# Z-yq/TensorflowASR

Hardware: AMD Instinct MI355X
Metric: audio-frames/sec/GPU + RTF, ConformerCTC(S) 10s utts, 1/2/4/8 MI355X (higher is better)
Workload: dtype f32

## Files before the change

### include/mi355asr.h

```cpp
#ifndef MI355ASR_H
#define MI355ASR_H

#include <stddef.h>
#include <stdint.h>

#ifdef __cplusplus
extern "C" {
#endif

#define MI355ASR_OK 0
#define MI355ASR_EINVAL -1
#define MI355ASR_ESTATE -2
#define MI355ASR_EWEIGHT -3
#define MI355ASR_EWORKSPACE -4
#define MI355ASR_EHIP -5

typedef struct mi355asr_model mi355asr_model;

typedef struct {
  int32_t dmodel;
  int32_t num_blocks;
  int32_t head_size;
  int32_t num_heads;
  int32_t kernel_size;
  float   fc_factor;
  int32_t reduction_factor;
  int32_t n_mels;
  int32_t sample_rate;
  int32_t stride_ms;
  int32_t n_dft;
  int32_t chunk_size;
  int32_t has_encoder;
  int32_t num_classes;
  int32_t ctc_num_blocks;
  int32_t ctc_kernel_size;
  float   ctc_fc_factor;
  int32_t gemm_dtype;
  int32_t mel_layer_type;
  int32_t add_wav_info;
} mi355asr_config;

const char* mi355asr_last_error(void);
const char* mi355asr_version(void);
int mi355asr_test_split_f16(const float* x_dev, int64_t n, uint16_t* hi_dev, uint16_t* lo_dev, void* stream);

int mi355asr_create(const mi355asr_config* cfg, mi355asr_model** out);
int mi355asr_destroy(mi355asr_model* m);

int mi355asr_load_weight(mi355asr_model* m, const char* name, const float* data_host, int32_t rank,
                         const int64_t* dims);
#define MI355ASR_DT_F32 0
#define MI355ASR_DT_F16 1
#define MI355ASR_DT_BF16 2
#define MI355ASR_DT_F64 3
#define MI355ASR_DT_I16 4
int mi355asr_load_weight_typed(mi355asr_model* m, const char* name, const void* data_host, int32_t dtype, int32_t rank,
                               const int64_t* dims);
int mi355asr_num_weights(const mi355asr_model* m);
const char* mi355asr_weight_name(const mi355asr_model* m, int32_t i);
int mi355asr_weight_shape(const mi355asr_model* m, int32_t i, int32_t* rank, int64_t* dims, int32_t max_rank);
int mi355asr_finalize_weights(mi355asr_model* m, void* stream);
int mi355asr_set_expected_rows(mi355asr_model* m, int64_t rows);
int mi355asr_stft_mode(const mi355asr_model* m);

int mi355asr_out_frames(const mi355asr_model* m, int32_t L, int32_t* mel_frames, int32_t* enc_frames);
int mi355asr_workspace_bytes(const mi355asr_model* m, int32_t B, int32_t L, size_t* bytes);
int mi355asr_ctc_workspace_bytes(const mi355asr_model* m, int32_t B, int32_t T, size_t* bytes);

int mi355asr_encoder_forward(mi355asr_model* m, const float* wav_dev, int32_t B, int32_t L, float* enc_out_dev,
                             void* ws_dev, size_t ws_bytes, void* stream);

int mi355asr_ctc_forward(mi355asr_model* m, const float* enc_dev, int32_t B, int32_t T, float* logits_dev,
                         int32_t* frame_argmax_dev, void* ws_dev, size_t ws_bytes, void* stream);

int mi355asr_ctc_greedy(const int32_t* frame_argmax_dev, const int32_t* in_len_dev, int32_t B, int32_t T,
                        int32_t blank, int32_t* ids_dev, int32_t* out_len_dev, void* stream);

// ... 249 lines not shown
```

### tensorflowasr_amd/_lib.py

```python
import ctypes
import os

_HERE = os.path.dirname(os.path.abspath(__file__))
LIB_PATH = os.environ.get("MI355ASR_LIB") or os.path.join(_HERE, "libmi355asr.so")


class Config(ctypes.Structure):
    _fields_ = [
        ("dmodel", ctypes.c_int32), ("num_blocks", ctypes.c_int32), ("head_size", ctypes.c_int32),
        ("num_heads", ctypes.c_int32), ("kernel_size", ctypes.c_int32), ("fc_factor", ctypes.c_float),
        ("reduction_factor", ctypes.c_int32), ("n_mels", ctypes.c_int32), ("sample_rate", ctypes.c_int32),
        ("stride_ms", ctypes.c_int32), ("n_dft", ctypes.c_int32), ("chunk_size", ctypes.c_int32),
        ("has_encoder", ctypes.c_int32), ("num_classes", ctypes.c_int32), ("ctc_num_blocks", ctypes.c_int32),
        ("ctc_kernel_size", ctypes.c_int32), ("ctc_fc_factor", ctypes.c_float), ("gemm_dtype", ctypes.c_int32),
        ("mel_layer_type", ctypes.c_int32), ("add_wav_info", ctypes.c_int32),
    ]


class ChunkConfig(ctypes.Structure):
    _fields_ = [(n, ctypes.c_int32) for n in ("dmodel", "head_size", "num_heads", "kernel_size")] + \
        [("fc_factor", ctypes.c_float)] + \
        [(n, ctypes.c_int32) for n in (
            "n_mels", "sample_rate", "stride_ms", "n_dft", "reduction_factor",
            "enc_num_blocks", "enc_win_front", "enc_win_back",
# ... 7 lines not shown
        [("fc_factor", ctypes.c_float), ("inp_classes", ctypes.c_int32), ("tar_classes", ctypes.c_int32)]


class VadConfig(ctypes.Structure):
    _fields_ = [(n, ctypes.c_int32) for n in ("dmodel", "frame", "decimate")]


class ChunkOutputs(ctypes.Structure):
    _fields_ = [(n, ctypes.c_void_p) for n in ("front_out", "enc_out", "picker_logits", "picker_hidden", "picked",
                                               "helper_out", "text_logits", "text_argmax")]


class ChunkStreamsOutputs(ctypes.Structure):
    _fields_ = [(n, ctypes.c_void_p) for n in ("phone_argmax", "n_picked", "text_argmax", "n_valid", "n_unvalid",
                                               "phone_logits", "text_logits", "picker_hidden")]


class BeamStreamsOutputs(ctypes.Structure):
    _fields_ = [(n, ctypes.c_void_p) for n in ("ids", "lens", "scores", "n_hyp", "frames", "status")]


class Mi355AsrError(RuntimeError):
    pass


_P = ctypes.c_void_p
_I = ctypes.c_int32
_SZ = ctypes.c_size_t

SIGNATURES = {
    "mi355asr_last_error": (ctypes.c_char_p, []),
    "mi355asr_version": (ctypes.c_char_p, []),
    "mi355asr_test_split_f16": (ctypes.c_int, [_P, ctypes.c_int64, _P, _P, _P]),
    "mi355asr_create": (ctypes.c_int, [ctypes.POINTER(Config), ctypes.POINTER(_P)]),
    "mi355asr_destroy": (ctypes.c_int, [_P]),
    "mi355asr_load_weight": (ctypes.c_int, [_P, ctypes.c_char_p, _P, _I, ctypes.POINTER(ctypes.c_int64)]),
    "mi355asr_load_weight_typed": (ctypes.c_int, [_P, ctypes.c_char_p, _P, _I, _I, ctypes.POINTER(ctypes.c_int64)]),
    "mi355asr_ctc_prefix_beam_workspace_bytes": (ctypes.c_int, [_I, _I, _I, _I, _I, ctypes.POINTER(ctypes.c_size_t)]),
    "mi355asr_frame_argmax": (ctypes.c_int, [_P, _I, _I, _P, _P]),
    "mi355asr_feature_pick_count": (ctypes.c_int, [_P, _I, _I, _I, _P, _P, _P, _P]),
    "mi355asr_feature_pick_gather": (ctypes.c_int, [_P, _P, _P, _P, _I, _I, _I, _I, _I, _P, _P, _P]),
    "mi355asr_num_weights": (ctypes.c_int, [_P]),
    "mi355asr_stft_mode": (ctypes.c_int, [_P]),
    "mi355asr_weight_name": (ctypes.c_char_p, [_P, _I]),
    "mi355asr_weight_shape": (ctypes.c_int, [_P, _I, ctypes.POINTER(ctypes.c_int32), ctypes.POINTER(ctypes.c_int64), _I]),
    "mi355asr_finalize_weights": (ctypes.c_int, [_P, _P]),
    "mi355asr_set_expected_rows": (ctypes.c_int, [_P, ctypes.c_int64]),
    "mi355asr_out_frames": (ctypes.c_int, [_P, _I, ctypes.POINTER(_I), ctypes.POINTER(_I)]),
    "mi355asr_workspace_bytes": (ctypes.c_int, [_P, _I, _I, ctypes.POINTER(_SZ)]),
    "mi355asr_ctc_workspace_bytes": (ctypes.c_int, [_P, _I, _I, ctypes.POINTER(_SZ)]),
    "mi355asr_encoder_forward": (ctypes.c_int, [_P, _P, _I, _I, _P, _P, _SZ, _P]),
    "mi355asr_ctc_forward": (ctypes.c_int, [_P, _P, _I, _I, _P, _P, _P, _SZ, _P]),
    "mi355asr_ctc_greedy": (ctypes.c_int, [_P, _P, _I, _I, _I, _P, _P, _P]),
    "mi355asr_ctc_loss_workspace_bytes": (ctypes.c_int, [_I, _I, _I, _I, _I, ctypes.POINTER(_SZ)]),
    "mi355asr_ctc_loss": (ctypes.c_int, [_P, _I, _P, _P, _P, _I, _I, _I, _I, _I, _P, _P, _P, _SZ, _P]),
    "mi355asr_ctc_align_workspace_bytes": (ctypes.c_int, [_I, _I, _I, _I, ctypes.POINTER(_SZ)]),
    "mi355asr_ctc_align": (ctypes.c_int, [_P, _I, _P, _P, _P, _I, _I, _I, _I, _I, _P, _P, _P, _P, _SZ, _P]),
    "mi355asr_ctc_prefix_beam_host": (ctypes.c_int, [_P, _P, _I, _I, _I, _I, ctypes.c_double, _I, _I, _I, _P, _P, _P, _P]),
    "mi355asr_ctc_prefix_beam": (ctypes.c_int, [_P, _I, _P, _I, _I, _I, _I, ctypes.c_double, _I, _I, _I, _P, _P, _P, _P,
                                                _P, _SZ, _P]),
    "mi355asr_beam_last_path": (_I, []),
    "mi355asr_beam_device_limits": (ctypes.c_int, [_I, ctypes.POINTER(_I), ctypes.POINTER(_I), ctypes.POINTER(_I), ctypes.POINTER(_I)]),
    "mi355asr_beam_math_eval": (ctypes.c_int, [_I, _P, _P, _I, _P]),
    "mi355asr_beam_create": (ctypes.c_int, [_I, _I, ctypes.c_double, _I, ctypes.POINTER(_P)]),
    "mi355asr_beam_decode": (ctypes.c_int, [_P, _P, _I, _I, _P, _P, _P, _P]),
    "mi355asr_beam_reset": (ctypes.c_int, [_P]),
# ... 84 lines not shown
```

### tensorflowasr_amd/csrc/api.hip

```cpp
#include "common.h"
#include "model.h"

namespace mi355 {


thread_local char g_err[512] = "";

int fail(int code, const char* fmt, ...) {
  va_list ap;
  va_start(ap, fmt);
  vsnprintf(g_err, sizeof(g_err), fmt, ap);
  va_end(ap);
  return code;
}

void same_pad(int n, int k, int s, int* out, int* before) {
  const int o = ceil_div(n, s);
  const int tot = std::max((o - 1) * s + k - n, 0);
  *out = o;
  *before = tot / 2;
}

int launch_mel_auto(const mi355asr_model* m, MelArgs& me, hipStream_t s) {
  if (m->mel_band) {
// ... 32 lines not shown
  p.amax = take(M);
  const int FT = ceil_div(F, 16);
  p.logp = take((size_t)Bp * F * m->dm.LP);
  p.pmax = take((size_t)Bp * std::max(FT * m->dm.NCH_dft, F));
  p.umax = take(Bp);
  p.mel = take((size_t)Bp * F * m->cfg.n_mels);
  p.sub = take(M * m->dm.F2 * d);
  p.wv_floats = wavpick_floats(m, Bp, F * m->dm.hop);
  p.wv = p.wv_floats ? take(p.wv_floats) : 0;
  p.total = lay.o;
  return p;
}


int geometry(const mi355asr_model* m, int B, int L, Geometry* g) {
  const auto& c = m->cfg;
  if (B <= 0 || L <= 0) return fail(MI355ASR_EINVAL, "B and L must be positive (B=%d, L=%d)", B, L);
  g->nblk = 1;
  g->Lb = L;
  if (c.chunk_size > 0) {
    if (L % c.chunk_size != 0)
      return fail(MI355ASR_EINVAL, "streaming encoder: L=%d is not a multiple of chunk_size=%d "
                  "(the reference reshapes [B,L,1]->[-1,chunk,1], conformer_blocks.py:585)", L, c.chunk_size);
    g->nblk = L / c.chunk_size;
    g->Lb = c.chunk_size;
  }
  g->Bp = B * g->nblk;
  g->F = ceil_div(g->Lb, m->dm.hop);
  g->T1 = ceil_div(g->F, m->dm.st1);
  g->T = ceil_div(g->T1, 2);
  return 0;
}


int run_mel(const mi355asr_model* m, const float* wav, int Bp, int Lb, int F, float* logp, float* pmax,
            float* umax, float* mel, hipStream_t s, const int32_t* wav_len = nullptr) {
  const auto& c = m->cfg;
  if (wav_len && (c.mel_layer_type != 0 || !m->fft_ok))
    return fail(MI355ASR_EINVAL, "ragged batches: the Melspectrogram frontend on the FFT STFT only (%s)",
                c.mel_layer_type == 1 ? "LEAF frontend" : c.mel_layer_type == 2 ? "Spectrogram layer" : "dense DFT STFT, stft_mode 0");
  if (c.mel_layer_type == 1) {
    int nf, pl;
    same_pad(Lb, 401, m->dm.hop, &nf, &pl);
    const int tile = m->leaf_terms ? kLeafSplitTile : 128, nrel = m->leaf_terms ? kLeafSplitSlots : 4;
    const int NH = ceil_div(Lb, tile);
    if (m->leaf_terms) {
      LeafConvArgs la{wav, m->leaf_wsplit, m->leaf_gcoef, logp, m->leaf_p0, m->leaf_p1, Bp, Lb, F, NH, m->dm.hop, pl};
      PROF(MI355ASR_K_STFT);
      LAUNCH_TRY(launch_leaf_conv_pool_split(m->leaf_terms, la, s), "leaf gabor conv (split bf16) + pooling");
    } else {
      LeafConvArgs la{wav, m->leaf_wp, m->leaf_gcoef, logp, m->leaf_p0, m->leaf_p1, Bp, Lb, F, NH, m->dm.hop, pl};
      PROF(MI355ASR_K_STFT);
      LAUNCH_TRY(launch_leaf_conv_pool(la, s), "leaf gabor conv + pooling");
    }
    LeafPcenArgs lp{logp, m->leaf_alpha, m->leaf_delta, m->leaf_root, m->leaf_smooth, m->leaf_gamma, m->leaf_beta, mel,
                    Bp, F, NH, m->dm.hop, pl, tile, nrel};
    { PROF(MI355ASR_K_MEL); LAUNCH_TRY(launch_leaf_pcen_norm(lp, s), "leaf PCEN + instance norm"); }
    return 0;
  }
  const int FT = ceil_div(F, 16);
  int out, before;
  same_pad(Lb, c.n_dft, m->dm.hop, &out, &before);
  StftArgs st{};
  st.wav = wav; st.logp = logp; st.pmax = pmax; st.wp = m->dft_wp;
  st.B = Bp; st.L = Lb; st.F = F; st.hop = m->dm.hop; st.pad_left = before; st.n_dft = c.n_dft;
  st.NT = m->dm.NT_dft; st.LP = m->dm.LP; st.nbins = m->dm.nbins; st.FT = FT; st.NCH = m->dm.NCH_dft;
  st.db10 = 1;
  int npart = FT * m->dm.NCH_dft;
  if (m->fft_ok) {
    FftStftArgs fa{wav, logp, pmax, m->fft_w1p, m->fft_w2p, m->fft_twc, m->fft_tws, m->fft_win,
                   Bp, Lb, F, m->dm.hop, before, m->dm.LP, 1};
    fa.w1s = m->fft_w1s; fa.w2s = m->fft_w2s; fa.w1h = m->fft_w1h; fa.w2h = m->fft_w2h;
    fa.wav_len = wav_len;
    { PROF(MI355ASR_K_STFT); LAUNCH_TRY(launch_fft_stft(fa, s), "stft (fft)"); }
    npart = F;
  } else {
    PROF(MI355ASR_K_STFT);
    LAUNCH_TRY(launch_stft(st, s), "stft");
  }
  UttMaxArgs um{pmax, umax, npart};
  um.wav_len = wav_len; um.hop = m->dm.hop;
  { PROF(MI355ASR_K_UTT_MAX); LAUNCH_TRY(launch_utt_max(um, Bp, s), "utterance max"); }
  MelArgs me{};
  me.logp = logp; me.umax = umax; me.mel = mel; me.wp = m->mel_wp;
  me.B = Bp; me.F = F; me.LP = m->dm.LP; me.nbins = m->dm.nbins; me.KBm = m->dm.KBm; me.NTm = m->dm.NTm;
  me.NM = c.n_mels; me.FT = FT; me.floor_db = -80.0f;
  if (c.mel_layer_type == 2) { PROF(MI355ASR_K_MEL); LAUNCH_TRY(launch_db_norm(me, s), "dB (Spectrogram layer)"); }
  else { PROF(MI355ASR_K_MEL); LAUNCH_TRY(launch_mel_auto(m, me, s), "dB + mel"); }
  return 0;
}

int run_subsampling(const mi355asr_model* m, const float* mel, int Bp, int F, float* sub, float* out,
                    hipStream_t s, bool mel_bounded, bool* defer_dense, const int32_t* wav_len) {
  if (defer_dense) *defer_dense = false;
  const auto& c = m->cfg;
  const int d = c.dmodel;
  int T1, pt1, T2, pt2;
  same_pad(F, 3, m->dm.st1, &T1, &pt1);
  same_pad(T1, 3, 2, &T2, &pt2);
  SubConvArgs sa{};
  sa.mel = mel; sa.out = sub;
  subconv_weights(m, sa, true);
  static const bool force_half = mi355_env("MI355ASR_SUBCONV_TERMS", -1) == 22;
  if (m->c2_whalf && (mel_bounded || force_half)) { sa.w2h = m->c2_whalf; sa.h_scale = m->c2_hscale; sa.h_wscale = m->c2_wscale; }
  if (sa.w2h && mel_bounded) { sa.c1_mscale = m->c1_mscale; sa.c1_wscale = m->c1_wscale; }
  sa.B = Bp; sa.F = F; sa.NM = c.n_mels; sa.T1 = T1; sa.F1 = m->dm.F1; sa.T2 = T2; sa.F2 = m->dm.F2;
// ... 244 lines not shown


}

thread_local int mi355asr_last_scheme = SCHEME_F32;

__global__ void split_f16_probe_kernel(const float* __restrict__ x, int64_t n, uint16_t* __restrict__ hi, uint16_t* __restrict__ lo) {
  const int64_t i = 2 * ((int64_t)blockIdx.x * blockDim.x + threadIdx.x);
  if (i >= n) return;
  const bool two = i + 1 < n;
  const float a = x[i], b = two ? x[i + 1] : 0.f;
  const unsigned h = split_hi_f16(a, b), l = split_lo_f16(h, a, b);
  hi[i] = (uint16_t)(h & 0xffffu);
  lo[i] = (uint16_t)(l & 0xffffu);
  if (two) {
    hi[i + 1] = (uint16_t)(h >> 16);
    lo[i + 1] = (uint16_t)(l >> 16);
  }
}

extern "C" {

const char* mi355asr_last_error(void) { return g_err; }
const char* mi355asr_version(void) { return "mi355asr 0.1 (gfx950, fp32 operands as fp16 pairs / bf16 triples on the MFMA pipe)"; }

int mi355asr_test_split_f16(const float* x_dev, int64_t n, uint16_t* hi_dev, uint16_t* lo_dev, void* stream) {
  if (!x_dev || !hi_dev || !lo_dev) return fail(MI355ASR_EINVAL, "null pointer");
  if (n < 1 || n > (int64_t)1 << 31) return fail(MI355ASR_EINVAL, "test_split_f16: need 1 <= n <= 2^31 (got %lld)", (long long)n);
  const int64_t pairs = (n + 1) / 2;
  hipLaunchKernelGGL(split_f16_probe_kernel, dim3((unsigned)((pairs + 255) / 256)), dim3(256), 0, (hipStream_t)stream, x_dev, n, hi_dev, lo_dev);
  return hipGetLastError() == hipSuccess ? MI355ASR_OK : fail(MI355ASR_EHIP, "test_split_f16: launch failed");
}

int mi355asr_create(const mi355asr_config* cfg, mi355asr_model** out) {
  if (!cfg || !out) return fail(MI355ASR_EINVAL, "null argument");
  mi355asr_config c = *cfg;
  if (c.mel_layer_type == 2) c.n_mels = c.n_dft / 2 + 1;
  if (c.dmodel != 144 && (c.dmodel % 128 != 0 || c.dmodel < 128 || c.dmodel > 1024))
    return fail(MI355ASR_EINVAL, "dmodel=%d: supported are 144 (ConformerS), 256 (ConformerM / StreamingS) and other multiples of 128 up to 1024 (512 = ConformerL)", c.dmodel);
  if (c.num_heads * c.head_size != c.dmodel)
    return fail(MI355ASR_EINVAL, "num_heads*head_size (%d*%d) must equal dmodel (%d)", c.num_heads, c.head_size, c.dmodel);
  if (!attention_head_size_ok(c.head_size))
    return fail(MI355ASR_EINVAL, "head_size=%d: attention kernels are instantiated for 12, 16, 24, 32, 36, 48, 64, 72 and 128", c.head_size);
  if (c.kernel_size < 1 || c.kernel_size > 1024)
    return fail(MI355ASR_EINVAL, "kernel_size=%d: must be in 1 .. 1024", c.kernel_size);
  if (c.num_classes > 0 && (c.ctc_kernel_size < 1 || c.ctc_kernel_size > 1024))
    return fail(MI355ASR_EINVAL, "ctc_kernel_size=%d: must be in 1 .. 1024", c.ctc_kernel_size);
  if (c.reduction_factor != 2 && c.reduction_factor != 4 && c.reduction_factor != 6 && c.reduction_factor != 8)
    return fail(MI355ASR_EINVAL, "reduction_factor=%d: 2, 4, 6 or 8 (conv1 time stride 1 .. 4)", c.reduction_factor);
  if (c.mel_layer_type < 0 || c.mel_layer_type > 2)
    return fail(MI355ASR_EINVAL, "mel_layer_type=%d: 0 (Melspectrogram), 1 (leaf) or 2 (Spectrogram)", c.mel_layer_type);
  if (c.mel_layer_type == 1 && (c.n_mels != 80 || c.stride_ms * c.sample_rate / 1000 != 160 || c.sample_rate != 16000))
    return fail(MI355ASR_EINVAL, "leaf frontend: instantiated for 80 filters, 16 kHz, 10 ms stride (window 401, hop 160)");
  if (c.gemm_dtype != 0 && c.gemm_dtype != 1) return fail(MI355ASR_EINVAL, "gemm_dtype=%d: 0 (fp32 MFMA) or 1 (bf16 MFMA)", c.gemm_dtype);
  if (c.n_dft != 1024) return fail(MI355ASR_EINVAL, "n_dft=%d: the reference hard-codes 1024 (conformer_blocks.py:312)", c.n_dft);
  if (c.mel_layer_type != 2 && c.n_mels != 80 && c.n_mels != 128)
    return fail(MI355ASR_EINVAL, "n_mels=%d: mel kernel instantiated for 80 and 128", c.n_mels);
  if (c.num_blocks < 0 || c.ctc_num_blocks < 0 || c.chunk_size < 0 || c.num_classes < 0)
    return fail(MI355ASR_EINVAL, "negative count in config");
  auto* m = new mi355asr_model();
  m->cfg = c;
  {
    const int t = (int)mi355_env("MI355ASR_LEAF_TERMS", -1);
    if (t == 0 || t == 2 || t == 3) m->leaf_terms = t;
  }
  Dims& dm = m->dm;
// ... 344 lines not shown
```

### tensorflowasr_amd/csrc/fft_stft.hip

```cpp
#include <cstdlib>
#include <type_traits>

#include "common.h"
#include "env.h"
#include "launch.h"

namespace {

constexpr int LDW = 36;

__global__ __launch_bounds__(BLOCK_THREADS, 2) void fft_stft_kernel(FftStftArgs a) {
  __shared__ float lds[WAVES_PER_BLOCK][2][32 * LDW];
  const int lane = threadIdx.x & 63;
  const int g = lane >> 4, g4 = g * 4, c = lane & 15;
  const int wave = threadIdx.x >> 6;
  float* Lre = lds[wave][0];
  float* Lim = lds[wave][1];
  const int wid = blockIdx.x * WAVES_PER_BLOCK + wave;
  const int nwaves = gridDim.x * WAVES_PER_BLOCK;
  const int total = a.B * a.F;

  const f32x4* __restrict__ w1p = reinterpret_cast<const f32x4*>(a.w1p) + lane;
  const f32x4* __restrict__ w2p = reinterpret_cast<const f32x4*>(a.w2p) + lane;
  f32x4 w1[2][4], w2[4][2];
// ... 152 lines not shown
}
DEV f32x4 mma32(u32x4_t a, u32x4_t b, f32x4 c) {
  return __builtin_amdgcn_mfma_f32_16x16x32_bf16(__builtin_bit_cast(bf16x8_t, a), __builtin_bit_cast(bf16x8_t, b), c, 0, 0, 0);
}
typedef _Float16 f16x8_t __attribute__((ext_vector_type(8)));
constexpr float kStageScale = 16384.f;
DEV Split8 split8h(f32x4 lo, f32x4 hi) {
  unsigned d0[4], d1[4];
  split8_f16(lo, hi, d0, d1);
  Split8 f;
  f.t[0] = u32x4_t{d0[0], d0[1], d0[2], d0[3]};
  f.t[1] = u32x4_t{d1[0], d1[1], d1[2], d1[3]};
  f.t[2] = u32x4_t{0u, 0u, 0u, 0u};
  return f;
}
DEV f32x4 mma32h(u32x4_t a, u32x4_t b, f32x4 c) {
  return __builtin_amdgcn_mfma_f32_16x16x32_f16(__builtin_bit_cast(f16x8_t, a), __builtin_bit_cast(f16x8_t, b), c, 0, 0, 0);
}
DEV float pow2_scale(float m) {
  const int e = (int)((__builtin_bit_cast(unsigned, m) >> 23) & 255u);
  return __builtin_bit_cast(float, (unsigned)(127 + min(100, max(-14, 140 - e))) << 23);
}
DEV float recip_pow2(float s) { return __builtin_bit_cast(float, 0x7f000000u - __builtin_bit_cast(unsigned, s)); }
DEV float max8(f32x4 a, f32x4 b) {
  return fmaxf(fmaxf(fmaxf(fabsf(a.x), fabsf(a.y)), fmaxf(fabsf(a.z), fabsf(a.w))), fmaxf(fmaxf(fabsf(b.x), fabsf(b.y)), fmaxf(fabsf(b.z), fabsf(b.w))));
}
template <int N> DEV float dpp_ror(float v) {
  return __builtin_bit_cast(float, __builtin_amdgcn_update_dpp(0, __builtin_bit_cast(int, v), 0x120 + N, 0xf, 0xf, false));
}
DEV float row_sum16(float v) { v += dpp_ror<8>(v); v += dpp_ror<4>(v); v += dpp_ror<2>(v); v += dpp_ror<1>(v); return v; }
DEV float row_max16(float v) {
  v = fmaxf(v, dpp_ror<8>(v)); v = fmaxf(v, dpp_ror<4>(v)); v = fmaxf(v, dpp_ror<2>(v)); return fmaxf(v, dpp_ror<1>(v));
}
DEV float col_max(float m) {
  return group_max(m);
}

#ifndef MI355ASR_STFT_DIAG
#define MI355ASR_STFT_DIAG 0
#endif
constexpr int FDG = MI355ASR_STFT_DIAG;
#ifndef MI355ASR_STFT_TABS_LDS
#define MI355ASR_STFT_TABS_LDS 1
#endif
template <int TM>
__global__ __launch_bounds__(BLOCK_THREADS, (TM == 2 && MI355ASR_STFT_TABS_LDS) ? 3 : 2) void fft_stft_split_kernel(FftStftArgs a) {
  constexpr bool TL = TM == 2 && MI355ASR_STFT_TABS_LDS;
  __shared__ float lds[WAVES_PER_BLOCK][2][32 * LDW];
  __shared__ __attribute__((aligned(16))) f32x4 tabs[TL ? 12 : 1][TL ? 64 : 1];
  const int lane = threadIdx.x & 63;
  const int g = lane >> 4, g4 = g * 4, c = lane & 15;
  const int wave = threadIdx.x >> 6;
  float* Lre = lds[wave][0];
  float* Lim = lds[wave][1];
  const int wid = blockIdx.x * WAVES_PER_BLOCK + wave;
  const int nwaves = gridDim.x * WAVES_PER_BLOCK;
  const int total = a.B * a.F;

  const u32x4_t* __restrict__ w1p = reinterpret_cast<const u32x4_t*>(TM == 2 ? a.w1h : a.w1s) + lane;
  const u32x4_t* __restrict__ w2p = reinterpret_cast<const u32x4_t*>(TM == 2 ? a.w2h : a.w2s) + lane;
  u32x4_t w1[4][TM], w2[2][2][TM];
#pragma unroll
  for (int nt = 0; nt < 4; ++nt)
#pragma unroll
    for (int t = 0; t < TM; ++t) w1[nt][t] = w1p[(nt * TM + t) * 64];
#pragma unroll
  for (int st = 0; st < 2; ++st)
#pragma unroll
    for (int nt = 0; nt < 2; ++nt)
#pragma unroll
      for (int t = 0; t < TM; ++t) w2[st][nt][t] = w2p[((st * 2 + nt) * TM + t) * 64];
  f32x4 hw[TL ? 1 : 2][TL ? 1 : 2], twc[TL ? 1 : 2][TL ? 1 : 2], tws[TL ? 1 : 2][TL ? 1 : 2];
#pragma unroll
  for (int rt = 0; rt < 2; ++rt) {
    const int n2 = 16 * rt + c;
#pragma unroll
    for (int kb = 0; kb < 2; ++kb) {
      f32x4 h_, c_, s_;
      h_.x = a.window[32 * (16 * kb + g4 + 0) + n2];
      h_.y = a.window[32 * (16 * kb + g4 + 1) + n2];
      h_.z = a.window[32 * (16 * kb + g4 + 2) + n2];
      h_.w = a.window[32 * (16 * kb + g4 + 3) + n2];
      c_.x = a.tw_c[(16 * kb + g4 + 0) * 32 + n2]; s_.x = a.tw_s[(16 * kb + g4 + 0) * 32 + n2];
      c_.y = a.tw_c[(16 * kb + g4 + 1) * 32 + n2]; s_.y = a.tw_s[(16 * kb + g4 + 1) * 32 + n2];
      c_.z = a.tw_c[(16 * kb + g4 + 2) * 32 + n2]; s_.z = a.tw_s[(16 * kb + g4 + 2) * 32 + n2];
      c_.w = a.tw_c[(16 * kb + g4 + 3) * 32 + n2]; s_.w = a.tw_s[(16 * kb + g4 + 3) * 32 + n2];
      if constexpr (TL) {
        if (wave == 0) { tabs[(2 * rt + kb) * 3 + 0][lane] = h_; tabs[(2 * rt + kb) * 3 + 1][lane] = c_; tabs[(2 * rt + kb) * 3 + 2][lane] = s_; }
      } else {
        hw[rt][kb] = h_; twc[rt][kb] = c_; tws[rt][kb] = s_;
      }
    }
  }
  if constexpr (TL) __syncthreads();
  auto tab = [&](int rt, int kb, int which) -> f32x4 {
    if constexpr (TL) return tabs[(2 * rt + kb) * 3 + which][lane];
    else return which == 0 ? hw[rt][kb] : (which == 1 ? twc[rt][kb] : tws[rt][kb]);
  };
  const int L = a.L;
  auto mma6 = [&](auto& acc, const auto& w, const Split8 (&x)[2], auto NT_T) {
    constexpr int NT = decltype(NT_T)::value;
#pragma unroll
    for (int ord = TM - 1; ord >= 0; --ord)
#pragma unroll
      for (int p = 0; p <= ord; ++p)
#pragma unroll
        for (int nt = 0; nt < NT; ++nt)
#pragma unroll
          for (int rt = 0; rt < 2; ++rt)
            acc[rt][nt] = TM == 2 ? mma32h(w[nt][ord - p], x[rt].t[p], acc[rt][nt]) : mma32(w[nt][ord - p], x[rt].t[p], acc[rt][nt]);
  };

#pragma unroll 1
  for (int fidx = wid; fidx < total; fidx += nwaves) {
    const int b = fidx / a.F, f = fidx - b * a.F;
    const float* __restrict__ wav = a.wav + (size_t)b * L;
    int Lv = L, pl = a.pad_left;
    if (a.wav_len) {
      int fo;
      Lv = a.wav_len[b];
      ragged_same_pad(Lv, 1024, a.hop, &fo, &pl);
    }
    const int base = f * a.hop - pl;
    f32x4 raw[2][2];
    if (!(FDG & 1) && base >= 0 && base + 1024 <= Lv) {
      const float* __restrict__ wl = wav + base + 32 * g4 + c;
#pragma unroll
      for (int rt = 0; rt < 2; ++rt)
#pragma unroll
        for (int kb = 0; kb < 2; ++kb) {
          const float* p = wl + 512 * kb + 16 * rt;
          raw[rt][kb] = f32x4{p[0], p[32], p[64], p[96]};
        }
    } else {
#pragma unroll
      for (int rt = 0; rt < 2; ++rt)
#pragma unroll
        for (int kb = 0; kb < 2; ++kb) {
          const int s0 = base + 32 * (16 * kb + g4) + 16 * rt + c;
          const bool o0 = (unsigned)(s0) < (unsigned)Lv, o1 = (unsigned)(s0 + 32) < (unsigned)Lv;
          const bool o2 = (unsigned)(s0 + 64) < (unsigned)Lv, o3 = (unsigned)(s0 + 96) < (unsigned)Lv;
          f32x4 v;
          if constexpr (FDG & 1) v = f32x4{(float)(s0 & 7), (float)(s0 & 3), 1.f, (float)c};
          else { v.x = wav[o0 ? s0 : 0]; v.y = wav[o1 ? s0 + 32 : 0]; v.z = wav[o2 ? s0 + 64 : 0]; v.w = wav[o3 ? s0 + 96 : 0]; }
          v.x = o0 ? v.x : 0.f; v.y = o1 ? v.y : 0.f; v.z = o2 ? v.z : 0.f; v.w = o3 ? v.w : 0.f;
          raw[rt][kb] = v;
        }
    }
    Split8 xs[2];
    float un1[2];
#pragma unroll
    for (int rt = 0; rt < 2; ++rt) {
      f32x4 xf[2];
#pragma unroll
      for (int kb = 0; kb < 2; ++kb) xf[kb] = raw[rt][kb] * tab(rt, kb, 0);
      if constexpr (TM == 2) {
        const float sx = pow2_scale(col_max(max8(xf[0], xf[1])));
        un1[rt] = recip_pow2(sx * kStageScale);
        xs[rt] = split8h(xf[0] * splat4(sx), xf[1] * splat4(sx));
      } else {
        un1[rt] = 1.f;
        xs[rt] = split8(xf[0], xf[1]);
      }
    }
    f32x4 acc1[2][4];
#pragma unroll
    for (int rt = 0; rt < 2; ++rt)
#pragma unroll
      for (int nt = 0; nt < 4; ++nt) acc1[rt][nt] = splat4(0.f);
    mma6(acc1, w1, xs, std::integral_constant<int, 4>{});
    if constexpr (TM == 2) {
#pragma unroll
      for (int rt = 0; rt < 2; ++rt)
#pragma unroll
        for (int nt = 0; nt < 4; ++nt) acc1[rt][nt] = acc1[rt][nt] * splat4(un1[rt]);
    }
    float nyq = (g == 0) ? ((c & 1) ? -1.f : 1.f) * (acc1[0][0].x + acc1[1][0].x) : 0.f;
    nyq = row_sum16(nyq);
#pragma unroll
    for (int rt = 0; rt < 2; ++rt) {
      const int n2 = 16 * rt + c;
#pragma unroll
      for (int nr = 0; nr < 2; ++nr) {
        const f32x4 are = acc1[rt][nr], aim = acc1[rt][2 + nr];
        const f32x4 tc = tab(rt, nr, 1), ts = tab(rt, nr, 2);
        const f32x4 bre = are * tc + aim * ts;
        const f32x4 bim = aim * tc - are * ts;
        const int k1 = 16 * nr + g4;
        Lre[(k1 + 0) * LDW + n2] = bre.x; Lre[(k1 + 1) * LDW + n2] = bre.y;
        Lre[(k1 + 2) * LDW + n2] = bre.z; Lre[(k1 + 3) * LDW + n2] = bre.w;
        Lim[(k1 + 0) * LDW + n2] = bim.x; Lim[(k1 + 1) * LDW + n2] = bim.y;
        Lim[(k1 + 2) * LDW + n2] = bim.z; Lim[(k1 + 3) * LDW + n2] = bim.w;
      }
    }
    __builtin_amdgcn_fence(__ATOMIC_RELEASE, "wavefront");
    __builtin_amdgcn_s_waitcnt(0xc07f);
    __builtin_amdgcn_fence(__ATOMIC_ACQUIRE, "wavefront");
    f32x4 acc2[2][2];
#pragma unroll
    for (int rt = 0; rt < 2; ++rt) {
      acc2[rt][0] = splat4(0.f);
      acc2[rt][1] = splat4(0.f);
    }
    if constexpr (TM == 2) {
      f32x4 yr[2][2], yi[2][2];
      float sy[2];
#pragma unroll
      for (int rt = 0; rt < 2; ++rt) {
        const float* sr = Lre + (16 * rt + c) * LDW + g4;
        const float* si = Lim + (16 * rt + c) * LDW + g4;
        yr[rt][0] = *reinterpret_cast<const f32x4*>(sr); yr[rt][1] = *reinterpret_cast<const f32x4*>(sr + 16);
        yi[rt][0] = *reinterpret_cast<const f32x4*>(si); yi[rt][1] = *reinterpret_cast<const f32x4*>(si + 16);
        sy[rt] = pow2_scale(col_max(fmaxf(max8(yr[rt][0], yr[rt][1]), max8(yi[rt][0], yi[rt][1]))));
      }
      Split8 ys[2];
#pragma unroll
      for (int rt = 0; rt < 2; ++rt) ys[rt] = split8h(yr[rt][0] * splat4(sy[rt]), yr[rt][1] * splat4(sy[rt]));
      mma6(acc2, w2[0], ys, std::integral_constant<int, 2>{});
#pragma unroll
      for (int rt = 0; rt < 2; ++rt) ys[rt] = split8h(yi[rt][0] * splat4(sy[rt]), yi[rt][1] * splat4(sy[rt]));
      mma6(acc2, w2[1], ys, std::integral_constant<int, 2>{});
#pragma unroll
      for (int rt = 0; rt < 2; ++rt) {
        const f32x4 un = splat4(recip_pow2(sy[rt] * kStageScale));
        acc2[rt][0] = acc2[rt][0] * un;
        acc2[rt][1] = acc2[rt][1] * un;
      }
    } else {
#pragma unroll
      for (int st = 0; st < 2; ++st) {
        Split8 ys[2];
#pragma unroll
        for (int rt = 0; rt < 2; ++rt) {
          const float* src = (st == 0 ? Lre : Lim) + (16 * rt + c) * LDW + g4;
          ys[rt] = split8(*reinterpret_cast<const f32x4*>(src), *reinterpret_cast<const f32x4*>(src + 16));
        }
        mma6(acc2, w2[st], ys, std::integral_constant<int, 2>{});
      }
    }
    float mx = -INFINITY;
    float* orow = a.logp + ((size_t)b * a.F + f) * a.LP;
    const float kscale = a.db10 ? (10.0f * 0.69314718f / 2.30258509f) : (0.69314718f / 2.30258509f);
#pragma unroll
    for (int rt = 0; rt < 2; ++rt) {
      const f32x4 re = acc2[rt][0], im = acc2[rt][1];
      const f32x4 p = re * re + im * im;
      const float pv[4] = {p.x, p.y, p.z, p.w};
#pragma unroll
      for (int j = 0; j < 4; ++j) {
        const float l = (FDG & 8) ? pv[j] : __log2f(fmaxf(pv[j], 1e-10f)) * kscale;
        if constexpr (!(FDG & 2)) orow[16 * rt + c + 32 * (g4 + j)] = l;
        mx = fmaxf(mx, l);
      }
    }
    if (lane == 0) {
      const float l = __log2f(fmaxf(nyq * nyq, 1e-10f)) * kscale;
      orow[512] = l;
      mx = fmaxf(mx, l);
    }
    mx = col_max(row_max16(mx));
    if (lane == 0) a.pmax[fidx] = mx;
  }
}

}

int launch_fft_stft(const FftStftArgs& a, hipStream_t s) {
  const int total = a.B * a.F;
  const int waves = std::min(total, 4096);
  static const bool split = mi355_env("MI355ASR_FFT_SPLIT", 1) != 0;
  static const bool three = mi355_env("MI355ASR_FFT_TERMS", -1) == 3;
  if (split && a.w1h && a.w2h && !three) {
    note_scheme(SCHEME_F16X2);
    const int waves2 = MI355ASR_STFT_TABS_LDS ? std::min(total, 3072) : waves;
    hipLaunchKernelGGL(fft_stft_split_kernel<2>, dim3((waves2 + WAVES_PER_BLOCK - 1) / WAVES_PER_BLOCK), dim3(BLOCK_THREADS), 0, s, a);
    return 0;
  }
  if (split && a.w1s && a.w2s) {
    note_scheme(SCHEME_BF16X3);
    hipLaunchKernelGGL(fft_stft_split_kernel<3>, dim3((waves + WAVES_PER_BLOCK - 1) / WAVES_PER_BLOCK), dim3(BLOCK_THREADS), 0, s, a);
    return 0;
  }
  note_scheme(SCHEME_F32);
  hipLaunchKernelGGL(fft_stft_kernel, dim3((waves + WAVES_PER_BLOCK - 1) / WAVES_PER_BLOCK), dim3(BLOCK_THREADS), 0, s, a);
  return 0;
}
```

Baseline: 35.77 million.

## Restructure FFT STFT split kernel: swapped MMA operands, LDS weights, 32-bit addressing

In the f16x2 split STFT kernel, the first-stage MMA now runs with swapped operands so its result lands in the layout the second stage needs. The per-wave LDS transpose and its wait are replaced by lane permutes (permlane swaps, ds_bpermute) for the scales and the Nyquist sum. DFT weight fragments move from registers into shared LDS, raising the occupancy bound from 3 to 4 waves and scaling the grid to match. Wave addressing uses readfirstlane and 32-bit offsets to cut address arithmetic. A test hook entry point for the STFT log-power path is also added. The cost is more LDS reads per frame and more code complexity.

```diff
diff --git a/include/mi355asr.h b/include/mi355asr.h
--- a/include/mi355asr.h
+++ b/include/mi355asr.h
@@ -43,6 +43,8 @@
 const char* mi355asr_last_error(void);
 const char* mi355asr_version(void);
 int mi355asr_test_split_f16(const float* x_dev, int64_t n, uint16_t* hi_dev, uint16_t* lo_dev, void* stream);
+int mi355asr_test_stft_logp(mi355asr_model* m, const float* wav_dev, int32_t B, int32_t L, float* logp_dev, float* pmax_dev,
+                            void* stream);
 
 int mi355asr_create(const mi355asr_config* cfg, mi355asr_model** out);
 int mi355asr_destroy(mi355asr_model* m);
diff --git a/tensorflowasr_amd/_lib.py b/tensorflowasr_amd/_lib.py
--- a/tensorflowasr_amd/_lib.py
+++ b/tensorflowasr_amd/_lib.py
@@ -63,6 +63,7 @@
     "mi355asr_last_error": (ctypes.c_char_p, []),
     "mi355asr_version": (ctypes.c_char_p, []),
     "mi355asr_test_split_f16": (ctypes.c_int, [_P, ctypes.c_int64, _P, _P, _P]),
+    "mi355asr_test_stft_logp": (ctypes.c_int, [_P, _P, _I, _I, _P, _P, _P]),
     "mi355asr_create": (ctypes.c_int, [ctypes.POINTER(Config), ctypes.POINTER(_P)]),
     "mi355asr_destroy": (ctypes.c_int, [_P]),
     "mi355asr_load_weight": (ctypes.c_int, [_P, ctypes.c_char_p, _P, _I, ctypes.POINTER(ctypes.c_int64)]),
diff --git a/tensorflowasr_amd/csrc/api.hip b/tensorflowasr_amd/csrc/api.hip
--- a/tensorflowasr_amd/csrc/api.hip
+++ b/tensorflowasr_amd/csrc/api.hip
@@ -88,6 +88,17 @@
   return 0;
 }
 
+
+FftStftArgs same_fft_stft_args(const mi355asr_model* m, const float* wav, int Bp, int Lb, int F, float* logp, float* pmax,
+                               const int32_t* wav_len) {
+  int out, before;
+  same_pad(Lb, m->cfg.n_dft, m->dm.hop, &out, &before);
+  FftStftArgs fa{wav, logp, pmax, m->fft_w1p, m->fft_w2p, m->fft_twc, m->fft_tws, m->fft_win,
+                 Bp, Lb, F, m->dm.hop, before, m->dm.LP, 1};
+  fa.w1s = m->fft_w1s; fa.w2s = m->fft_w2s; fa.w1h = m->fft_w1h; fa.w2h = m->fft_w2h;
+  fa.wav_len = wav_len;
+  return fa;
+}
 
 int run_mel(const mi355asr_model* m, const float* wav, int Bp, int Lb, int F, float* logp, float* pmax,
             float* umax, float* mel, hipStream_t s, const int32_t* wav_len = nullptr) {
@@ -124,10 +135,7 @@
   st.db10 = 1;
   int npart = FT * m->dm.NCH_dft;
   if (m->fft_ok) {
-    FftStftArgs fa{wav, logp, pmax, m->fft_w1p, m->fft_w2p, m->fft_twc, m->fft_tws, m->fft_win,
-                   Bp, Lb, F, m->dm.hop, before, m->dm.LP, 1};
-    fa.w1s = m->fft_w1s; fa.w2s = m->fft_w2s; fa.w1h = m->fft_w1h; fa.w2h = m->fft_w2h;
-    fa.wav_len = wav_len;
+    const FftStftArgs fa = same_fft_stft_args(m, wav, Bp, Lb, F, logp, pmax, wav_len);
     { PROF(MI355ASR_K_STFT); LAUNCH_TRY(launch_fft_stft(fa, s), "stft (fft)"); }
     npart = F;
   } else {
@@ -438,6 +446,18 @@
   return hipGetLastError() == hipSuccess ? MI355ASR_OK : fail(MI355ASR_EHIP, "test_split_f16: launch failed");
 }
 
+int mi355asr_test_stft_logp(mi355asr_model* m, const float* wav_dev, int32_t B, int32_t L, float* logp_dev, float* pmax_dev, void* stream) {
+  if (int rc = check_ready(m, true)) return rc;
+  if (!wav_dev || !logp_dev || !pmax_dev || B <= 0 || L <= 0) return fail(MI355ASR_EINVAL, "bad argument");
+  if (!m->fft_ok || m->cfg.mel_layer_type == 1 || m->cfg.chunk_size > 0)
+    return fail(MI355ASR_EINVAL, "test_stft_logp: the SAME-padded front on the FFT STFT only");
+  const int F = ceil_div(L, m->dm.hop);
+  if ((int64_t)B * F > INT32_MAX) return fail(MI355ASR_EINVAL, "test_stft_logp: too many frames");
+  const FftStftArgs fa = same_fft_stft_args(m, wav_dev, B, L, F, logp_dev, pmax_dev, nullptr);
+  LAUNCH_TRY(launch_fft_stft(fa, (hipStream_t)stream), "stft (fft, test hook)");
+  return MI355ASR_OK;
+}
+
 int mi355asr_create(const mi355asr_config* cfg, mi355asr_model** out) {
   if (!cfg || !out) return fail(MI355ASR_EINVAL, "null argument");
   mi355asr_config c = *cfg;
diff --git a/tensorflowasr_amd/csrc/fft_stft.hip b/tensorflowasr_amd/csrc/fft_stft.hip
--- a/tensorflowasr_amd/csrc/fft_stft.hip
+++ b/tensorflowasr_amd/csrc/fft_stft.hip
@@ -208,6 +208,26 @@
 DEV float row_max16(float v) {
   v = fmaxf(v, dpp_ror<8>(v)); v = fmaxf(v, dpp_ror<4>(v)); v = fmaxf(v, dpp_ror<2>(v)); return fmaxf(v, dpp_ror<1>(v));
 }
+#ifndef MI355ASR_STFT_SWAP
+#define MI355ASR_STFT_SWAP 1
+#endif
+#ifndef MI355ASR_STFT_W_LDS
+#define MI355ASR_STFT_W_LDS 1
+#endif
+#ifndef MI355ASR_STFT_ADDR32
+#define MI355ASR_STFT_ADDR32 1
+#endif
+typedef unsigned u32x2_perm __attribute__((ext_vector_type(2)));
+DEV void rows_pair16(float v, float& x, float& y) {
+  const u32x2_perm r = __builtin_amdgcn_permlane16_swap(__builtin_bit_cast(unsigned, v), __builtin_bit_cast(unsigned, v), false, false);
+  const unsigned rx = r.x, ry = r.y;
+  x = __builtin_bit_cast(float, rx); y = __builtin_bit_cast(float, ry);
+}
+DEV void rows_pair32(float v, float& x, float& y) {
+  const u32x2_perm r = __builtin_amdgcn_permlane32_swap(__builtin_bit_cast(unsigned, v), __builtin_bit_cast(unsigned, v), false, false);
+  const unsigned rx = r.x, ry = r.y;
+  x = __builtin_bit_cast(float, rx); y = __builtin_bit_cast(float, ry);
+}
 DEV float col_max(float m) {
   return group_max(m);
 }
@@ -219,33 +239,43 @@
 #ifndef MI355ASR_STFT_TABS_LDS
 #define MI355ASR_STFT_TABS_LDS 1
 #endif
+constexpr int kStftWaves = MI355ASR_STFT_TABS_LDS == 0 ? 2 : (MI355ASR_STFT_SWAP != 0 && MI355ASR_STFT_W_LDS != 0) ? 4 : 3;
 template <int TM>
-__global__ __launch_bounds__(BLOCK_THREADS, (TM == 2 && MI355ASR_STFT_TABS_LDS) ? 3 : 2) void fft_stft_split_kernel(FftStftArgs a) {
+__global__ __launch_bounds__(BLOCK_THREADS, TM == 2 ? kStftWaves : 2) void fft_stft_split_kernel(FftStftArgs a) {
   constexpr bool TL = TM == 2 && MI355ASR_STFT_TABS_LDS;
-  __shared__ float lds[WAVES_PER_BLOCK][2][32 * LDW];
+  constexpr bool SW = TM == 2 && MI355ASR_STFT_SWAP;
+  constexpr bool WL = SW && TL && MI355ASR_STFT_W_LDS;
+  constexpr bool A32 = TM == 2 && MI355ASR_STFT_ADDR32;
+  __shared__ float lds[SW ? 1 : WAVES_PER_BLOCK][2][SW ? 1 : 32 * LDW];
   __shared__ __attribute__((aligned(16))) f32x4 tabs[TL ? 12 : 1][TL ? 64 : 1];
+  __shared__ __attribute__((aligned(16))) u32x4_t wfr[WL ? 16 : 1][WL ? 64 : 1];
   const int lane = threadIdx.x & 63;
   const int g = lane >> 4, g4 = g * 4, c = lane & 15;
   const int wave = threadIdx.x >> 6;
-  float* Lre = lds[wave][0];
-  float* Lim = lds[wave][1];
+  float* Lre = lds[SW ? 0 : wave][0];
+  float* Lim = lds[SW ? 0 : wave][1];
   const int wid = blockIdx.x * WAVES_PER_BLOCK + wave;
   const int nwaves = gridDim.x * WAVES_PER_BLOCK;
   const int total = a.B * a.F;
 
   const u32x4_t* __restrict__ w1p = reinterpret_cast<const u32x4_t*>(TM == 2 ? a.w1h : a.w1s) + lane;
   const u32x4_t* __restrict__ w2p = reinterpret_cast<const u32x4_t*>(TM == 2 ? a.w2h : a.w2s) + lane;
-  u32x4_t w1[4][TM], w2[2][2][TM];
-#pragma unroll
-  for (int nt = 0; nt < 4; ++nt)
-#pragma unroll
-    for (int t = 0; t < TM; ++t) w1[nt][t] = w1p[(nt * TM + t) * 64];
-#pragma unroll
-  for (int st = 0; st < 2; ++st)
-#pragma unroll
-    for (int nt = 0; nt < 2; ++nt)
-#pragma unroll
-      for (int t = 0; t < TM; ++t) w2[st][nt][t] = w2p[((st * 2 + nt) * TM + t) * 64];
+  u32x4_t w1[WL ? 1 : 4][TM], w2[WL ? 1 : 2][2][TM];
+  if constexpr (WL) {
+#pragma unroll
+    for (int i = 0; i < 4; ++i) wfr[4 * wave + i][lane] = wave < 2 ? w1p[(4 * wave + i) * 64] : w2p[(4 * wave + i - 8) * 64];
+  } else {
+#pragma unroll
+    for (int nt = 0; nt < 4; ++nt)
+#pragma unroll
+      for (int t = 0; t < TM; ++t) w1[nt][t] = w1p[(nt * TM + t) * 64];
+#pragma unroll
+    for (int st = 0; st < 2; ++st)
+#pragma unroll
+      for (int nt = 0; nt < 2; ++nt)
+#pragma unroll
+        for (int t = 0; t < TM; ++t) w2[st][nt][t] = w2p[((st * 2 + nt) * TM + t) * 64];
+  }
   f32x4 hw[TL ? 1 : 2][TL ? 1 : 2], twc[TL ? 1 : 2][TL ? 1 : 2], tws[TL ? 1 : 2][TL ? 1 : 2];
 #pragma unroll
   for (int rt = 0; rt < 2; ++rt) {
@@ -257,10 +287,15 @@
       h_.y = a.window[32 * (16 * kb + g4 + 1) + n2];
       h_.z = a.window[32 * (16 * kb + g4 + 2) + n2];
       h_.w = a.window[32 * (16 * kb + g4 + 3) + n2];
-      c_.x = a.tw_c[(16 * kb + g4 + 0) * 32 + n2]; s_.x = a.tw_s[(16 * kb + g4 + 0) * 32 + n2];
-      c_.y = a.tw_c[(16 * kb + g4 + 1) * 32 + n2]; s_.y = a.tw_s[(16 * kb + g4 + 1) * 32 + n2];
-      c_.z = a.tw_c[(16 * kb + g4 + 2) * 32 + n2]; s_.z = a.tw_s[(16 * kb + g4 + 2) * 32 + n2];
-      c_.w = a.tw_c[(16 * kb + g4 + 3) * 32 + n2]; s_.w = a.tw_s[(16 * kb + g4 + 3) * 32 + n2];
+      if constexpr (SW) {
+        c_ = ldg4(a.tw_c + (16 * kb + c) * 32 + 16 * rt + g4);
+        s_ = ldg4(a.tw_s + (16 * kb + c) * 32 + 16 * rt + g4);
+      } else {
+        c_.x = a.tw_c[(16 * kb + g4 + 0) * 32 + n2]; s_.x = a.tw_s[(16 * kb + g4 + 0) * 32 + n2];
+        c_.y = a.tw_c[(16 * kb + g4 + 1) * 32 + n2]; s_.y = a.tw_s[(16 * kb + g4 + 1) * 32 + n2];
+        c_.z = a.tw_c[(16 * kb + g4 + 2) * 32 + n2]; s_.z = a.tw_s[(16 * kb + g4 + 2) * 32 + n2];
+        c_.w = a.tw_c[(16 * kb + g4 + 3) * 32 + n2]; s_.w = a.tw_s[(16 * kb + g4 + 3) * 32 + n2];
+      }
       if constexpr (TL) {
         if (wave == 0) { tabs[(2 * rt + kb) * 3 + 0][lane] = h_; tabs[(2 * rt + kb) * 3 + 1][lane] = c_; tabs[(2 * rt + kb) * 3 + 2][lane] = s_; }
       } else {
@@ -269,13 +304,27 @@
     }
   }
   if constexpr (TL) __syncthreads();
+  int ll = lane;
   auto tab = [&](int rt, int kb, int which) -> f32x4 {
-    if constexpr (TL) return tabs[(2 * rt + kb) * 3 + which][lane];
+    if constexpr (TL) return tabs[(2 * rt + kb) * 3 + which][ll];
     else return which == 0 ? hw[rt][kb] : (which == 1 ? twc[rt][kb] : tws[rt][kb]);
   };
+  auto W1 = [&](int nt, int t) -> u32x4_t {
+    if constexpr (WL) return wfr[nt * 2 + t][ll];
+    else return w1[nt][t];
+  };
+  auto W2a = [&](int nt, int t) -> u32x4_t {
+    if constexpr (WL) return wfr[8 + nt * 2 + t][ll];
+    else return w2[0][nt][t];
+  };
+  auto W2b = [&](int nt, int t) -> u32x4_t {
+    if constexpr (WL) return wfr[12 + nt * 2 + t][ll];
+    else return w2[WL ? 0 : 1][nt][t];
+  };
   const int L = a.L;
-  auto mma6 = [&](auto& acc, const auto& w, const Split8 (&x)[2], auto NT_T) {
+  auto mma6 = [&](auto& acc, const auto& w, const Split8 (&x)[2], auto NT_T, auto SWAP_T) {
     constexpr int NT = decltype(NT_T)::value;
+    constexpr bool SWP = decltype(SWAP_T)::value;
 #pragma unroll
     for (int ord = TM - 1; ord >= 0; --ord)
 #pragma unroll
@@ -284,11 +333,15 @@
         for (int nt = 0; nt < NT; ++nt)
 #pragma unroll
           for (int rt = 0; rt < 2; ++rt)
-            acc[rt][nt] = TM == 2 ? mma32h(w[nt][ord - p], x[rt].t[p], acc[rt][nt]) : mma32(w[nt][ord - p], x[rt].t[p], acc[rt][nt]);
+            acc[rt][nt] = TM != 2 ? mma32(w(nt, ord - p), x[rt].t[p], acc[rt][nt])
+                          : SWP   ? mma32h(x[rt].t[p], w(nt, ord - p), acc[rt][nt]) : mma32h(w(nt, ord - p), x[rt].t[p], acc[rt][nt]);
   };
+  const unsigned lofs = 32 * g4 + c;
 
 #pragma unroll 1
-  for (int fidx = wid; fidx < total; fidx += nwaves) {
+  for (int fidx_ = wid; fidx_ < total; fidx_ += nwaves) {
+    const int fidx = A32 ? __builtin_amdgcn_readfirstlane(fidx_) : fidx_;
+    if constexpr (SW) asm volatile("" : "+v"(ll));
     const int b = fidx / a.F, f = fidx - b * a.F;
     const float* __restrict__ wav = a.wav + (size_t)b * L;
     int Lv = L, pl = a.pad_left;
@@ -300,14 +353,25 @@
     const int base = f * a.hop - pl;
     f32x4 raw[2][2];
     if (!(FDG & 1) && base >= 0 && base + 1024 <= Lv) {
-      const float* __restrict__ wl = wav + base + 32 * g4 + c;
-#pragma unroll
-      for (int rt = 0; rt < 2; ++rt)
-#pragma unroll
-        for (int kb = 0; kb < 2; ++kb) {
-          const float* p = wl + 512 * kb + 16 * rt;
-          raw[rt][kb] = f32x4{p[0], p[32], p[64], p[96]};
-        }
+      if constexpr (A32) {
+        const float* __restrict__ fb = wav + base;
+#pragma unroll
+        for (int rt = 0; rt < 2; ++rt)
+#pragma unroll
+          for (int kb = 0; kb < 2; ++kb) {
+            const unsigned o = lofs + 512u * kb + 16u * rt;
+            raw[rt][kb] = f32x4{fb[o], fb[o + 32u], fb[o + 64u], fb[o + 96u]};
+          }
+      } else {
+        const float* __restrict__ wl = wav + base + 32 * g4 + c;
+#pragma unroll
+        for (int rt = 0; rt < 2; ++rt)
+#pragma unroll
+          for (int kb = 0; kb < 2; ++kb) {
+            const float* p = wl + 512 * kb + 16 * rt;
+            raw[rt][kb] = f32x4{p[0], p[32], p[64], p[96]};
+          }
+      }
     } else {
 #pragma unroll
       for (int rt = 0; rt < 2; ++rt)
@@ -318,7 +382,10 @@
           const bool o2 = (unsigned)(s0 + 64) < (unsigned)Lv, o3 = (unsigned)(s0 + 96) < (unsigned)Lv;
           f32x4 v;
           if constexpr (FDG & 1) v = f32x4{(float)(s0 & 7), (float)(s0 & 3), 1.f, (float)c};
-          else { v.x = wav[o0 ? s0 : 0]; v.y = wav[o1 ? s0 + 32 : 0]; v.z = wav[o2 ? s0 + 64 : 0]; v.w = wav[o3 ? s0 + 96 : 0]; }
+          else if constexpr (A32) {
+            v.x = wav[(unsigned)(o0 ? s0 : 0)]; v.y = wav[(unsigned)(o1 ? s0 + 32 : 0)];
+            v.z = wav[(unsigned)(o2 ? s0 + 64 : 0)]; v.w = wav[(unsigned)(o3 ? s0 + 96 : 0)];
+          } else { v.x = wav[o0 ? s0 : 0]; v.y = wav[o1 ? s0 + 32 : 0]; v.z = wav[o2 ? s0 + 64 : 0]; v.w = wav[o3 ? s0 + 96 : 0]; }
           v.x = o0 ? v.x : 0.f; v.y = o1 ? v.y : 0.f; v.z = o2 ? v.z : 0.f; v.w = o3 ? v.w : 0.f;
           raw[rt][kb] = v;
         }
@@ -339,19 +406,51 @@
         xs[rt] = split8(xf[0], xf[1]);
       }
     }
+    f32x4 un4[2];
+    if constexpr (SW) {
+      const int pk = (int)(__builtin_bit_cast(unsigned, un1[1]) | (__builtin_bit_cast(unsigned, un1[0]) >> 23));
+#pragma unroll
+      for (int j = 0; j < 4; ++j) {
+        const unsigned q = (unsigned)__builtin_amdgcn_ds_bpermute(4 * (g4 + j), pk);
+        un4[0][j] = __builtin_bit_cast(float, q << 23);
+        un4[1][j] = __builtin_bit_cast(float, q & 0x7f800000u);
+      }
+    }
     f32x4 acc1[2][4];
 #pragma unroll
     for (int rt = 0; rt < 2; ++rt)
 #pragma unroll
       for (int nt = 0; nt < 4; ++nt) acc1[rt][nt] = splat4(0.f);
-    mma6(acc1, w1, xs, std::integral_constant<int, 4>{});
+    mma6(acc1, W1, xs, std::integral_constant<int, 4>{}, std::integral_constant<bool, SW>{});
     if constexpr (TM == 2) {
 #pragma unroll
       for (int rt = 0; rt < 2; ++rt)
 #pragma unroll
-        for (int nt = 0; nt < 4; ++nt) acc1[rt][nt] = acc1[rt][nt] * splat4(un1[rt]);
-    }
-    float nyq = (g == 0) ? ((c & 1) ? -1.f : 1.f) * (acc1[0][0].x + acc1[1][0].x) : 0.f;
+        for (int nt = 0; nt < 4; ++nt) acc1[rt][nt] = acc1[rt][nt] * (SW ? un4[rt] : splat4(un1[rt]));
+    }
+    float nyq;
+    f32x4 yr[2][2], yi[2][2];
+    if constexpr (SW) {
+      const f32x4 t4 = acc1[0][0] + acc1[1][0];
+      float u[4] = {t4.x, -t4.y, t4.z, -t4.w};
+#pragma unroll
+      for (int j = 0; j < 4; ++j) {
+        float x, y;
+        rows_pair32(u[j], x, y); u[j] = x + y;
+        rows_pair16(u[j], x, y); u[j] = x + y;
+      }
+      nyq = (u[0] + u[2]) + (u[1] + u[3]);
+#pragma unroll
+      for (int rt = 0; rt < 2; ++rt)
+#pragma unroll
+        for (int nr = 0; nr < 2; ++nr) {
+          const f32x4 are = acc1[rt][nr], aim = acc1[rt][2 + nr];
+          const f32x4 tc = tab(rt, nr, 1), ts = tab(rt, nr, 2);
+          yr[nr][rt] = are * tc + aim * ts;
+          yi[nr][rt] = aim * tc - are * ts;
+        }
+    } else {
+    nyq = (g == 0) ? ((c & 1) ? -1.f : 1.f) * (acc1[0][0].x + acc1[1][0].x) : 0.f;
     nyq = row_sum16(nyq);
 #pragma unroll
     for (int rt = 0; rt < 2; ++rt) {
@@ -372,30 +471,33 @@
     __builtin_amdgcn_fence(__ATOMIC_RELEASE, "wavefront");
     __builtin_amdgcn_s_waitcnt(0xc07f);
     __builtin_amdgcn_fence(__ATOMIC_ACQUIRE, "wavefront");
+    }
     f32x4 acc2[2][2];
 #pragma unroll
     for (int rt = 0; rt < 2; ++rt) {
       acc2[rt][0] = splat4(0.f);
       acc2[rt][1] = splat4(0.f);
     }
+    constexpr std::integral_constant<bool, false> NOSWAP{};
     if constexpr (TM == 2) {
-      f32x4 yr[2][2], yi[2][2];
       float sy[2];
 #pragma unroll
       for (int rt = 0; rt < 2; ++rt) {
-        const float* sr = Lre + (16 * rt + c) * LDW + g4;
-        const float* si = Lim + (16 * rt + c) * LDW + g4;
-        yr[rt][0] = *reinterpret_cast<const f32x4*>(sr); yr[rt][1] = *reinterpret_cast<const f32x4*>(sr + 16);
-        yi[rt][0] = *reinterpret_cast<const f32x4*>(si); yi[rt][1] = *reinterpret_cast<const f32x4*>(si + 16);
+        if constexpr (!SW) {
+          const float* sr = Lre + (16 * rt + c) * LDW + g4;
+          const float* si = Lim + (16 * rt + c) * LDW + g4;
+          yr[rt][0] = *reinterpret_cast<const f32x4*>(sr); yr[rt][1] = *reinterpret_cast<const f32x4*>(sr + 16);
+          yi[rt][0] = *reinterpret_cast<const f32x4*>(si); yi[rt][1] = *reinterpret_cast<const f32x4*>(si + 16);
+        }
         sy[rt] = pow2_scale(col_max(fmaxf(max8(yr[rt][0], yr[rt][1]), max8(yi[rt][0], yi[rt][1]))));
       }
       Split8 ys[2];
 #pragma unroll
       for (int rt = 0; rt < 2; ++rt) ys[rt] = split8h(yr[rt][0] * splat4(sy[rt]), yr[rt][1] * splat4(sy[rt]));
-      mma6(acc2, w2[0], ys, std::integral_constant<int, 2>{});
+      mma6(acc2, W2a, ys, std::integral_constant<int, 2>{}, NOSWAP);
 #pragma unroll
       for (int rt = 0; rt < 2; ++rt) ys[rt] = split8h(yi[rt][0] * splat4(sy[rt]), yi[rt][1] * splat4(sy[rt]));
-      mma6(acc2, w2[1], ys, std::integral_constant<int, 2>{});
+      mma6(acc2, W2b, ys, std::integral_constant<int, 2>{}, NOSWAP);
 #pragma unroll
       for (int rt = 0; rt < 2; ++rt) {
         const f32x4 un = splat4(recip_pow2(sy[rt] * kStageScale));
@@ -411,7 +513,8 @@
           const float* src = (st == 0 ? Lre : Lim) + (16 * rt + c) * LDW + g4;
           ys[rt] = split8(*reinterpret_cast<const f32x4*>(src), *reinterpret_cast<const f32x4*>(src + 16));
         }
-        mma6(acc2, w2[st], ys, std::integral_constant<int, 2>{});
+        if (st == 0) mma6(acc2, W2a, ys, std::integral_constant<int, 2>{}, NOSWAP);
+        else mma6(acc2, W2b, ys, std::integral_constant<int, 2>{}, NOSWAP);
       }
     }
     float mx = -INFINITY;
@@ -425,7 +528,10 @@
 #pragma unroll
       for (int j = 0; j < 4; ++j) {
         const float l = (FDG & 8) ? pv[j] : __log2f(fmaxf(pv[j], 1e-10f)) * kscale;
-        if constexpr (!(FDG & 2)) orow[16 * rt + c + 32 * (g4 + j)] = l;
+        if constexpr (!(FDG & 2)) {
+          if constexpr (A32) orow[lofs + 16u * rt + 32u * j] = l;
+          else orow[16 * rt + c + 32 * (g4 + j)] = l;
+        }
         mx = fmaxf(mx, l);
       }
     }
@@ -448,7 +554,7 @@
   static const bool three = mi355_env("MI355ASR_FFT_TERMS", -1) == 3;
   if (split && a.w1h && a.w2h && !three) {
     note_scheme(SCHEME_F16X2);
-    const int waves2 = MI355ASR_STFT_TABS_LDS ? std::min(total, 3072) : waves;
+    const int waves2 = MI355ASR_STFT_TABS_LDS ? std::min(total, 1024 * kStftWaves) : waves;
     hipLaunchKernelGGL(fft_stft_split_kernel<2>, dim3((waves2 + WAVES_PER_BLOCK - 1) / WAVES_PER_BLOCK), dim3(BLOCK_THREADS), 0, s, a);
     return 0;
   }
```

New measurement: 35.94 million (median of 6 runs). About the same (+0.5%).
